# zenlc2000/pycuda-euler

Measured on AMD Instinct MI355X. Metric: k-mers/sec (encode+hash+deBruijn+Euler), 10Mx100bp k=31, 1/2/4/8 GPU, higher is better.
Workload: dtype u64

## Files before the change

### pycuda-euler_amd/csrc/assemble.hip

```cpp
#include "common.h"
#include "count_global.h"
#include "graph.h"

#include <rocprim/rocprim.hpp>

#include <algorithm>
#include <cmath>
#include <climits>
#include <cstring>
#include <cstddef>
#include <functional>
#include <type_traits>
#include <vector>

#include "count_part.h"
#include "count_v2.h"
#include "count_sk2.h"
#include "shard.h"
#include "compact.h"
#include "count_wide.h"
#include "hostin.h"
#include "join_w.h"
#include "extended.h"
#include "rank_tile.h"
// ... 166 lines not shown
    PinnedVec<uint8_t> h_lc8;
    PinnedVec<uint32_t> h_links32;
    bool links_compact = false;
    HostBuf h_blk;
    bool want_dict = false;
    hipEvent_t ev[2 * EC_NSTAGES] = {};
    hipEvent_t kev[2 * EC_NKERNELS] = {};
    bool kused[EC_NKERNELS] = {};
    bool sused[EC_NSTAGES] = {};
    bool events = false;
    bool timing = false;
    bool stage_timing = false;
    unsigned int n_dense = 0;
    bool dense_ok = false;
    bool stats_ok = false;
    unsigned flags = 0;
    DevBuf ocnt, rbc, mbid, mbid2, midx, midx2, gcur, cwalk, ewalk, lc8;
    bool no_index = false;
    uint64_t shard_base = 0;
    const uint64_t *lc_off = nullptr;
    uint64_t lc_n = 0, lc_L = 0;
    DevBuf bnp;
    DevBuf fcur, bb2;
    DevBuf nrec;
    SolidIndex gidx{};
    SolidIndexW gidxw{};
    bool graph_loaded = false;
    bool placed = false;
    uint64_t seg_lo = 0, seg_Ur = 0;
    DevBuf jrec, joid, jout, jseg, jcnt;
    DevBuf xrec;
    DevBuf skm_rec, skm_ev, skm_end;
    DevBuf wcodes_tab;
    HostBuf hmeta;
    int owner_rule = 0;
    bool own_valid = false;
    int own_rule = 0, own_nowners = 0;
    unsigned int own_n = 0, own_nblk = 0;
    std::vector<unsigned int> own_hi;
    hipStream_t cstream = nullptr;
    struct Pipe {
        bool active = false;
        bool packed = false;
        int nchunks = 0, done = 0;
        std::vector<uint64_t> blo, bhi;
        std::vector<uint64_t> ravail;
        std::vector<uint64_t> elo, ehi;
        uint64_t first_len = 0;
        const uint32_t *codes = nullptr;
        const uint64_t *exc_pos = nullptr;
        const uint8_t *exc_byte = nullptr;
        uint8_t *ascii = nullptr;
        std::vector<hipEvent_t> ev;
    } pipe;
    DevBuf p_codes, p_exc;
    struct Staged {
        Pipe pipe;
        DevBuf codes, exc, off;
        hipEvent_t free_ev = nullptr;
        uint64_t nreads = 0, nbases = 0;
    } stg[2];
    int stg_head = 0, stg_n = 0;
    bool xalpha = false;
    XAlpha xa{};
    DevBuf x_par, x_irr, x_in, x_succ, x_done, x_lk, x_lv, x_lk2, x_lv2, x_len, x_m, x_cid, x_head, x_tail;
    DevBuf jl_kof, jl_rs, jl_re, jl_cnt, jl_off, jl_flag;
    DevBuf rpack;
    DevBuf rt_tcnt, rt_tbase, rt_srec, rt_snrec, rt_sidx, rt_pks, rt_rks, rt_hasp, rt_lr;
    int spec_rounds = 0;
    DevBuf wbv;
    uint64_t seg_n0 = 0, seg_n1 = 0;
    struct Pending {
        int kind = 0;
        uint64_t n = 0;
        unsigned int ntiles = 0;
        bool planned = false;
    } hold;
    SuperRec *chain_scr = nullptr;
    unsigned int seg_nc = 0;
    uint64_t seg_nchars = 0;
    DevBuf run_cnt, run_ends, run_dends;
    DevBuf rt_lb;
    unsigned long long lb_epoch = 0;
    uint64_t run_nr = 0, run_nch = 0, run_nends = 0;
    bool runs_ready = false;
    int part_stage = 0;
    bool clip_ok = false;
    const char *clip_why = "a new session holds no assembly";
    SolidIndex cidx{};
    SolidIndexW cidxw{};
    DevBuf clip_cand, clip_list, clip_kill, clip_tot;
    DevBuf pop_key, pop_sum, pop_tcnt, pop_toff, pop_tile;
    DevBuf spec_hist;
};

static const char *const CLIP_WHY_STEPWISE =
    "the last calls were stepwise ones (ec_count_shard / ec_merge_owned* / ec_graph_*), which leave no one-GPU assembly";

static inline void drop_step_state(ec_session *s) {
    s->hold.kind = 0;
    s->runs_ready = false;
    s->chain_scr = nullptr;
    s->part_stage = 0;
}

namespace {
constexpr size_t BOUNCE_CAP = 64 << 10, BOUNCE_MAX = 16 << 10;

int d2h(ec_session *s, void *dst, const void *src, size_t n, hipStream_t st) {
    if (!n) return EC_OK;
    const size_t off = (s->bused + 15) & ~size_t(15);
    if (n > BOUNCE_MAX || off + n > BOUNCE_CAP) {
        EC_HIP(hipMemcpyAsync(dst, src, n, hipMemcpyDeviceToHost, st));
        return EC_OK;
    }
    if (!s->bounce.p) EC_CHECK(s->bounce.resize(BOUNCE_CAP));
    EC_HIP(hipMemcpyAsync(s->bounce.p + off, src, n, hipMemcpyDeviceToHost, st));
    s->pend.push_back({dst, off, n});
    s->bused = off + n;
    return EC_OK;
}

int host_wait(ec_session *s, hipEvent_t ev) {
    const hipError_t e = hipEventSynchronize(ev);
    for (const auto &q : s->pend) std::memcpy(q.dst, s->bounce.p + q.off, q.n);
    s->pend.clear();
    s->bused = 0;
    if (e != hipSuccess) {
        set_error("HIP error %s", hipGetErrorString(e));
        return EC_ERR_HIP;
    }
    return EC_OK;
}

int host_sync(ec_session *s, hipStream_t st) {
    const hipError_t e = hipStreamSynchronize(st);
    for (const auto &q : s->pend) std::memcpy(q.dst, s->bounce.p + q.off, q.n);
    s->pend.clear();
    s->bused = 0;
    if (e != hipSuccess) {
        set_error("HIP error %s", hipGetErrorString(e));
        return EC_ERR_HIP;
    }
    return EC_OK;
}
}

namespace ec {

template <typename Ops>
__global__ void __launch_bounds__(256) k_kmers_to_agg(const char *chars, const unsigned int *counts, uint64_t n, int k,
                                                      typename RecOf<typename Ops::K>::T *out, unsigned long long *bad) {
    using K = typename Ops::K;
    const K mask = Ops::mask(k);
    for (uint64_t t = blockIdx.x * (uint64_t)blockDim.x + threadIdx.x; t < n; t += (uint64_t)gridDim.x * blockDim.x) {
        const char *x = chars + t * (uint64_t)k;
        K code{};
        bool ok = true;
        for (int i = 0; i < k; i++) {
            const uint32_t b = base_code((unsigned char)x[i]);
            ok &= b < 4;
            code = Ops::push(code, b & 3u, mask);
        }
        if (!ok) atomicMin(bad, (unsigned long long)t);
        const K tw = Ops::twin(code, k);
        out[t] = RecOf<K>::make(code < tw ? code : tw, code <= tw ? counts[t] : 0u,
// ... 2036 lines not shown
    const unsigned int *SIDX = sidx ? sidx : s->rt_sidx.as<unsigned int>();
    const size_t cap = std::max<size_t>(M, 1);
    EC_CHECK(s->rt_snrec.ensure(cap * sizeof(SNodeRec)));
    EC_CHECK(s->rt_hasp.ensure(cap));
    EC_CHECK(s->rt_pks.ensure(cap * 4));
    EC_CHECK(s->rt_rks.ensure(cap * 4));
    EC_CHECK(s->rid.ensure(cap * 8));
    EC_CHECK(s->rlist.ensure(cap * 4));
    EC_CHECK(s->nextR.ensure(cap * 4));
    EC_CHECK(s->st0.ensure(cap * sizeof(RJump)));
    EC_CHECK(s->st1.ensure(cap * sizeof(RJump)));
    EC_CHECK(s->rbc.ensure(((cap + RULER_CHUNK - 1) / RULER_CHUNK) * 8 + 8));
    SNodeRec *snrec = s->rt_snrec.as<SNodeRec>();
    if (!pre_init) EC_HIP(hipMemsetAsync(s->rt_hasp.p, 0, M, st));
    k_super_link<<<grid_for(M, B), B, 0, st>>>(srec, M, SIDX, snrec, s->rt_hasp.as<uint8_t>());
    if (!pre_init) {
        EC_HIP(hipMemsetAsync(s->rid.p, 0xFF, (size_t)M * 8, st));
        EC_HIP(hipMemsetAsync(&dsc->nr, 0, 4, st));
        EC_HIP(hipMemsetAsync(&dsc->nvisited, 0, 8, st));
    }
    const unsigned int masks[4] = {15u, 3u, 1u, 0u};
    unsigned int r0 = 0;
    const unsigned int nblk = (M + RULER_CHUNK - 1) / RULER_CHUNK;
    for (int it = 0; it < 4; it++) {
        k_srulers_count<<<nblk, B, 0, st>>>(s->rt_hasp.as<uint8_t>(), M, masks[it], it == 0, s->rid.as<uint2>(),
                                            s->rbc.as<unsigned int>());
        EC_CHECK(scan_incl_u32(s, s->rbc.as<unsigned int>(), s->rbc.as<unsigned int>() + nblk, nblk));
        k_srulers<<<nblk, B, 0, st>>>(s->rt_hasp.as<uint8_t>(), M, masks[it], it == 0, s->rbc.as<unsigned int>() + nblk,
                                      &dsc->nr, s->rid.as<uint2>(), s->rlist.as<unsigned int>());
        k_rulers_total<<<1, 1, 0, st>>>(s->rbc.as<unsigned int>() + nblk, nblk, &dsc->nr);
        k_walk_s<<<2048, B, 0, st>>>(snrec, s->rlist.as<unsigned int>(), r0, &dsc->nr, masks[it], s->rid.as<uint2>(),
                                     s->nextR.as<unsigned int>(), s->st0.as<RJump>(), &dsc->nvisited, srec);
        EC_CHECK(d2h(s, &hsc, dsc, sizeof(Scalars), st));
        EC_CHECK(host_sync(s, st));
        r0 = hsc.nr;
        if (hsc.nvisited >= M) break;
    }
    nr = hsc.nr;
    if (hsc.nvisited != M) {
        set_error("ruling set covered %llu of %u chains", (unsigned long long)hsc.nvisited, M);
        return EC_ERR_STATE;
    }
    k_rjump_init<<<grid_for(nr, B), B, 0, st>>>(s->nextR.as<unsigned int>(), nr, s->st0.as<RJump>());
    rounds = 1;
    while ((1ull << (rounds - 1)) < (unsigned long long)nr) rounds++;
    rounds = std::min(rounds + 1, 63);
    RJump *bufs[2] = {s->st0.as<RJump>(), s->st1.as<RJump>()};
    EC_HIP(hipMemsetAsync(dsc->active, 0, sizeof(dsc->active), st));
    for (int r = 0; r < rounds; r++)
        k_rjump<<<grid_for(nr, B), B, 0, st>>>(bufs[r & 1], bufs[(r + 1) & 1], nr, N, r ? &dsc->active[r - 1] : nullptr,
                                              &dsc->active[r], &dsc->final_sel, (unsigned)((r + 1) & 1));
    k_finalize_s<<<grid_for(M, B), B, 0, st>>>(snrec, srec, s->rid.as<uint2>(), s->rlist.as<unsigned int>(), bufs[0],
                                              bufs[1], &dsc->final_sel, &dsc->active[rounds - 1], M,
                                              s->rt_pks.as<unsigned int>(), s->rt_rks.as<unsigned int>(),
                                              s->PL.as<unsigned int>(), s->PM.as<unsigned long long>());
    k_cycle_len_s<<<grid_for(nr, B), B, 0, st>>>(s->nextR.as<unsigned int>(), s->rlist.as<unsigned int>(), srec, bufs[0],
                                                bufs[1], &dsc->final_sel, &dsc->active[rounds - 1], nr,
                                                s->PL.as<unsigned int>(), s->PM.as<unsigned long long>());
    return EC_OK;
}

int rank_supers_async(ec_session *s, unsigned int N, const unsigned long long *dM, int &rounds,
                      unsigned int mcap = 0, const unsigned int *sidx = nullptr) {
    const unsigned int G = mcap ? mcap : N;
    hipStream_t st = s->stream;
    const unsigned B = 256;
    Scalars *dsc = s->scal.as<Scalars>();
    SuperRec *srec = s->rt_srec.as<SuperRec>();
    const size_t cap = mcap ? (size_t)mcap + 4096 : std::max<size_t>(N, 1);
    const unsigned int spare = mcap ? 16u : 0u;
    EC_CHECK(s->rt_snrec.ensure(cap * sizeof(SNodeRec), spare));
    EC_CHECK(s->rt_pks.ensure(cap * 4, spare));
    EC_CHECK(s->rt_rks.ensure(cap * 4, spare));
    EC_CHECK(s->rlist.ensure(cap * 4, spare));
    EC_CHECK(s->nextR.ensure(cap * 4, spare));
    EC_CHECK(s->rbc.ensure(((cap + RULER_CHUNK - 1) / RULER_CHUNK) * 8 + 8, spare));
    SNodeRec *snrec = s->rt_snrec.as<SNodeRec>();
    const unsigned int *dnr = &dsc->nr;
    const unsigned int gs = std::min(grid_for(G, B), 4096u);
    k_super_link<<<gs, B, 0, st>>>(srec, 0, sidx ? sidx : s->rt_sidx.as<unsigned int>(), snrec,
                                   s->rt_hasp.as<uint8_t>(), dM);
    const unsigned int smask = 15u;
    const unsigned int nblk = (G + RULER_CHUNK - 1) / RULER_CHUNK;
    k_srulers_count<<<nblk, B, 0, st>>>(s->rt_hasp.as<uint8_t>(), 0, smask, 1, s->rid.as<uint2>(),
                                        s->rbc.as<unsigned int>(), dM);
    EC_CHECK(scan_incl_u32(s, s->rbc.as<unsigned int>(), s->rbc.as<unsigned int>() + nblk, nblk));
    k_srulers<<<nblk, B, 0, st>>>(s->rt_hasp.as<uint8_t>(), 0, smask, 1, s->rbc.as<unsigned int>() + nblk, &dsc->nr,
                                  s->rid.as<uint2>(), s->rlist.as<unsigned int>(), dM);
    k_rulers_total<<<1, 1, 0, st>>>(s->rbc.as<unsigned int>() + nblk, nblk, &dsc->nr);
    k_walk_s<<<2048, B, 0, st>>>(snrec, s->rlist.as<unsigned int>(), 0, &dsc->nr, smask, s->rid.as<uint2>(),
                                 s->nextR.as<unsigned int>(), s->st0.as<RJump>(), &dsc->nvisited, srec);
    const unsigned int gr = std::min(grid_for(G / 8u + 1, B), 2048u);
    k_rjump_init<<<gr, B, 0, st>>>(s->nextR.as<unsigned int>(), 0, s->st0.as<RJump>(), dnr);
    rounds = 1;
    while ((1ull << (rounds - 1)) < (unsigned long long)G) rounds++;
    rounds = std::min(rounds + 1, 63);
    if (s->spec_rounds > 0 && s->spec_rounds < rounds) rounds = s->spec_rounds;
    RJump *bufs[2] = {s->st0.as<RJump>(), s->st1.as<RJump>()};
    for (int r = 0; r < rounds; r++)
        k_rjump<<<gr, B, 0, st>>>(bufs[r & 1], bufs[(r + 1) & 1], 0, N, r ? &dsc->active[r - 1] : nullptr,
                                  &dsc->active[r], &dsc->final_sel, (unsigned)((r + 1) & 1), dnr);
    k_finalize_s<<<gs, B, 0, st>>>(snrec, srec, s->rid.as<uint2>(), s->rlist.as<unsigned int>(), bufs[0], bufs[1],
                                   &dsc->final_sel, &dsc->active[rounds - 1], 0, s->rt_pks.as<unsigned int>(),
                                   s->rt_rks.as<unsigned int>(), s->PL.as<unsigned int>(),
                                   s->PM.as<unsigned long long>(), dM);
    k_cycle_len_s<<<gr, B, 0, st>>>(s->nextR.as<unsigned int>(), s->rlist.as<unsigned int>(), srec, bufs[0], bufs[1],
                                    &dsc->final_sel, &dsc->active[rounds - 1], 0, s->PL.as<unsigned int>(),
                                    s->PM.as<unsigned long long>(), dnr);
    return EC_OK;
}

__global__ void __launch_bounds__(256) k_pack_chars(const uint4 *chars, const unsigned long long *total, uint64_t cap16,
                                                    uint32_t *codes) {
    const uint64_t n16 = min<uint64_t>((*total + 15) / 16, cap16);
    for (uint64_t t = blockIdx.x * (uint64_t)blockDim.x + threadIdx.x; t < n16; t += (uint64_t)gridDim.x * blockDim.x) {
        const uint4 v = chars[t];
        const uint32_t w[4] = {v.x, v.y, v.z, v.w};
        uint32_t out = 0;
#pragma unroll
        for (int u = 0; u < 4; u++) {
            const uint32_t x = ((w[u] >> 1) ^ (w[u] >> 2)) & 0x03030303u;
            const uint32_t y = x | (x >> 6);
            out |= ((y | (y >> 12)) & 0xFFu) << (8 * u);
        }
        codes[t] = out;
    }
}

constexpr unsigned int OCOPY_MIN = 1u << 16;
int rounds_used(const Scalars &h, int rounds) {
    if (rounds <= 0 || h.active[rounds - 1]) return 0;
    int used = 1;
    for (int r = 0; r < rounds; r++)
        if (h.active[r]) used = r + 2;
    return std::min(used, rounds);
}
void note_rounds(ec_session *s, const Scalars &h, int rounds) {
    const int used = rounds_used(h, rounds);
    s->spec_rounds = used ? used + 1 : 0;
}

int x_cut(ec_session *s, unsigned int U, unsigned int &nx) {
    hipStream_t st = s->stream;
    const unsigned B = 256;
    Scalars *dsc = s->scal.as<Scalars>();
    const unsigned int N = 2 * U;
    nx = 0;
    EC_HIP(hipMemsetAsync(&dsc->nasym, 0, 16, st));
    k_x_asym<<<grid_for(N, B), B, 0, st>>>(s->upal.as<uint8_t>(), s->succ.as<unsigned int>(), N, &dsc->nasym);
    unsigned int nasym = 0;
    EC_CHECK(d2h(s, &nasym, &dsc->nasym, 4, st));
    EC_CHECK(host_sync(s, st));
    if (kn().verbose) fprintf(stderr, "extended: %u one-way links among %u nodes\n", nasym, N);
    if (!nasym) return EC_OK;
    EC_CHECK(s->x_par.ensure((size_t)U * 4));
    EC_CHECK(s->x_irr.ensure(U));
    EC_CHECK(s->x_in.ensure(U));
    EC_CHECK(s->x_succ.ensure((size_t)N * 4));
    EC_CHECK(s->x_lk.ensure((size_t)N * 8));
    EC_CHECK(s->x_lk2.ensure((size_t)N * 8));
    EC_CHECK(s->x_lv.ensure((size_t)N * 4));
    EC_CHECK(s->x_lv2.ensure((size_t)N * 4));
    unsigned int *par = s->x_par.as<unsigned int>(), *tree = s->x_lv2.as<unsigned int>();
    k_x_iota<<<grid_for(U, B), B, 0, st>>>(tree, U);
    k_x_uf_link<<<grid_for(N, B), B, 0, st>>>(s->upal.as<uint8_t>(), s->succ.as<unsigned int>(), N, tree);
    k_x_uf_flatten<<<grid_for(U, B), B, 0, st>>>(U, tree, par);
    EC_HIP(hipMemsetAsync(s->x_irr.p, 0, U, st));
    k_x_mark_irr<<<grid_for(N, B), B, 0, st>>>(s->upal.as<uint8_t>(), s->succ.as<unsigned int>(), N, par,
                                              s->x_irr.as<uint8_t>());
    k_x_cut<<<grid_for(N, B), B, 0, st>>>(s->upal.as<uint8_t>(), N, par, s->x_irr.as<uint8_t>(), s->x_in.as<uint8_t>(),
                                         s->succ.as<unsigned int>(), s->x_succ.as<unsigned int>(),
                                         s->dfc.as<unsigned long long>(), s->dft.as<unsigned long long>(),
// ... 1223 lines not shown
    for (uint64_t i = 0; i < n_exc; i++)
        if (exc_pos[i] >= nbases || (i && exc_pos[i] <= exc_pos[i - 1])) {
            set_error("exception %llu: position %llu not ascending inside [0, %llu)", (unsigned long long)i,
                      (unsigned long long)exc_pos[i], (unsigned long long)nbases);
            return EC_ERR_ARG;
        }
    return EC_OK;
}

int stage_packed(ec_session *s, Pipe &pp, DevBuf &codes_b, DevBuf &exc_b, DevBuf &off_b, hipEvent_t after,
                 const uint8_t *codes, uint64_t nbases, const uint64_t *offsets, uint64_t nreads, uint32_t read_len,
                 const uint64_t *exc_pos, const uint8_t *exc_byte, uint64_t n_exc) {
    const uint64_t ncodes = (nbases + 3) / 4;
    EC_CHECK(off_b.ensure((nreads + 1) * 8));
    EC_CHECK(codes_b.ensure(((ncodes + 3) & ~3ull) + 16));
    EC_CHECK(exc_b.ensure(n_exc * 9 + 16));
    EC_CHECK(pipe_plan(s, pp, nbases, 1, offsets, nreads, read_len, after));
    pp.packed = true;
    pp.first_len = nreads ? (offsets ? offsets[1] - offsets[0] : read_len) : 0;
    pp.codes = codes_b.as<uint32_t>();
    pp.exc_pos = exc_b.as<uint64_t>();
    pp.exc_byte = exc_b.as<uint8_t>() + n_exc * 8;
    if (n_exc) {
        EC_HIP(hipMemcpyAsync(exc_b.p, exc_pos, n_exc * 8, hipMemcpyHostToDevice, s->cstream));
        EC_HIP(hipMemcpyAsync(exc_b.as<uint8_t>() + n_exc * 8, exc_byte, n_exc, hipMemcpyHostToDevice, s->cstream));
    }
    if (!offsets)
        k_iota_off<<<grid_for(nreads + 1, 256, 16384), 256, 0, s->cstream>>>(off_b.as<uint64_t>(), nreads + 1, read_len);
    for (int c = 0; c < pp.nchunks; c++) {
        const uint64_t c0 = pp.blo[c] / 4, c1 = c + 1 == pp.nchunks ? ncodes : pp.bhi[c] / 4;
        if (c1 > c0)
            EC_HIP(hipMemcpyAsync(codes_b.as<uint8_t>() + c0, codes + c0, c1 - c0, hipMemcpyHostToDevice, s->cstream));
        if (offsets) EC_CHECK(pipe_copy_offsets(s, pp, c, offsets, off_b.as<uint64_t>()));
        pp.elo[c] = (uint64_t)(std::lower_bound(exc_pos, exc_pos + n_exc, pp.blo[c]) - exc_pos);
        pp.ehi[c] = (uint64_t)(std::lower_bound(exc_pos, exc_pos + n_exc, pp.bhi[c]) - exc_pos);
        EC_HIP(hipEventRecord(pp.ev[c], s->cstream));
    }
    return EC_OK;
}

}

static void unpack_codes(const uint8_t *codes, uint64_t n, char *out) {
    static const struct Lut {
        uint32_t v[256];
        Lut() {
            const char acgt[4] = {'A', 'C', 'G', 'T'};
            for (int b = 0; b < 256; b++) {
                uint32_t w = 0;
                for (int j = 0; j < 4; j++) w |= (uint32_t)(uint8_t)acgt[(b >> (2 * j)) & 3] << (8 * j);
                v[b] = w;
            }
        }
    } lut;
    auto run = [&](uint64_t b0, uint64_t b1) {
        for (uint64_t i = b0; i < b1; i++) memcpy(out + 4 * i, &lut.v[codes[i]], 4);
    };
    const uint64_t full = n / 4;
    const unsigned nt = full >= (1ull << 20) ? std::max(1u, std::min(16u, std::thread::hardware_concurrency())) : 1u;
    if (nt > 1) {
        std::vector<std::thread> th;
        for (unsigned t = 0; t < nt; t++) th.emplace_back(run, full * t / nt, full * (t + 1) / nt);
        for (auto &x : th) x.join();
    } else {
        run(0, full);
    }
    for (uint64_t c = 4 * full; c < n; c++) out[c] = "ACGT"[(codes[full] >> (2 * (c & 3))) & 3];
}

template <typename Fn>
static void for_each_buf(ec_session *s, Fn fn) {
    DevBuf *all[] = {&s->h_reads, &s->h_offsets, &s->hll, &s->scal, &s->table, &s->dkey, &s->dcnt, &s->dfc, &s->dft,
                     &s->upal, &s->outdeg, &s->cand, &s->succ, &s->pred, &s->st0, &s->st1, &s->startOf, &s->skeys,
                     &s->svals, &s->skeys2, &s->svals2, &s->cidxOf, &s->clen, &s->coff, &s->chars, &s->cfirst,
                     &s->clast, &s->headOf, &s->tailOf, &s->lk, &s->lcnt, &s->tmp, &s->dchars, &s->dcounts,
                     &s->rid, &s->rlist, &s->nextR, &s->PK, &s->RK, &s->PL, &s->PM,
                     &s->ocnt, &s->hist, &s->ftot, &s->cnt, &s->offs, &s->bstart, &s->tot, &s->recs, &s->recs2, &s->sub, &s->bnp, &s->rbc,
                     &s->mbid, &s->mbid2, &s->midx, &s->midx2, &s->gcur, &s->cwalk, &s->ewalk, &s->lc8, &s->x_par, &s->x_irr,
                     &s->x_in, &s->x_succ, &s->x_done, &s->x_lk, &s->x_lv, &s->x_lk2, &s->x_lv2, &s->x_len,
                     &s->x_m, &s->x_cid, &s->x_head, &s->x_tail, &s->rt_tcnt, &s->rt_tbase, &s->rt_srec,
                     &s->rt_snrec, &s->rt_sidx, &s->rt_pks, &s->rt_rks, &s->rt_hasp, &s->rt_lr, &s->wbv, &s->bmark, &s->rt_tb,
                     &s->jrec, &s->joid, &s->jout, &s->jseg, &s->jcnt, &s->xrec,
                     &s->skm_rec, &s->skm_ev, &s->skm_end, &s->wcodes_tab,
                     &s->run_cnt, &s->run_ends, &s->run_dends, &s->rt_lb,
                     &s->jl_kof, &s->jl_rs, &s->jl_re, &s->jl_cnt, &s->jl_off, &s->jl_flag, &s->jl_frec, &s->rpack,
                     &s->clip_cand, &s->clip_list, &s->clip_kill, &s->clip_tot,
                     &s->pop_key, &s->pop_sum, &s->pop_tcnt, &s->pop_toff, &s->pop_tile, &s->spec_hist};
    for (auto *b : all) fn(*b);
}

extern "C" {

int ec_session_create(ec_session **out, int device) {
    if (!out) {
        set_error("null out");
        return EC_ERR_ARG;
    }
    int n = 0;
    EC_HIP(hipGetDeviceCount(&n));
    if (device < 0 || device >= n) {
        set_error("device %d not in [0,%d)", device, n);
        return EC_ERR_ARG;
    }
    EC_HIP(hipSetDevice(device));
    ec_session *s = new ec_session();
    s->device = device;
    if (hipStreamCreateWithFlags(&s->stream, hipStreamNonBlocking) != hipSuccess) {
        delete s;
        set_error("hipStreamCreate failed");
        return EC_ERR_HIP;
    }
    s->own_stream = true;
    *out = s;
    return EC_OK;
}

int ec_session_set_stream(ec_session *s, void *hip_stream) {
    if (!s) return EC_ERR_ARG;
    EC_HIP(hipSetDevice(s->device));
    if (hip_stream == EC_OWN_STREAM) {
        if (!s->own_stream) {
            EC_HIP(hipStreamCreateWithFlags(&s->stream, hipStreamNonBlocking));
            s->own_stream = true;
        }
        return EC_OK;
    }
    if (s->own_stream && s->stream) {
        (void)host_sync(s, s->stream);
        hipStreamDestroy(s->stream);
    }
    s->own_stream = false;
    s->stream = (hipStream_t)hip_stream;
    return EC_OK;
}

uint64_t ec_session_bytes(ec_session *s) {
    uint64_t n = 0;
    if (s) for_each_buf(s, [&](DevBuf &b) { n += b.cap; });
    return n;
}

int ec_session_trim(ec_session *s, uint64_t min_bytes) {
    if (!s) return EC_ERR_ARG;
    EC_HIP(hipSetDevice(s->device));
    if (s->stream) EC_HIP(hipStreamSynchronize(s->stream));
    if (s->ostream) EC_HIP(hipStreamSynchronize(s->ostream));
    if (s->cstream) EC_HIP(hipStreamSynchronize(s->cstream));
    for_each_buf(s, [&](DevBuf &b) {
        if (b.cap >= min_bytes && &b != &s->scal) b.release();
    });
    drop_step_state(s);
    s->n_dense = 0;
    s->dense_ok = false;
    s->clip_ok = false;
    s->clip_why = "ec_session_trim released the assembly's device state";
    s->own_valid = false;
    s->bmark_ok = false;
    s->seg_marks = 0;
    s->skspec.valid = false;
    s->jlspec.valid = s->jlspec.queued = false;
    s->graph_loaded = false;
    s->placed = false;
    s->pipe.active = false;
    return EC_OK;
}

int ec_mem_stats(uint64_t *held, uint64_t *peak, int reset) {
// ... 1402 lines not shown
```

### pycuda-euler_amd/csrc/graph.h

```cpp
#pragma once
#include "count_global.h"
#include "count_part.h"
#include "superkmer.h"
#include "wide.h"

namespace ec {

struct SolidIndex {
    const Slot *table;
    uint64_t capmask;
    const SubSlot *sub;
    int bbits;
    unsigned int slots;
    int sk;
    const uint8_t *npb;
    int pmax;
    MinCfg mc;
    int bijk = 0;
    __device__ inline unsigned int find_in(uint64_t c, unsigned int h, uint64_t b) const {
        const SubSlot *r = sub + b * slots;
        unsigned int n = slots;
        if (npb) {
            n = slots >> pmax;
            r += ((h >> 11) & ((1u << npb[b]) - 1)) * n;
// ... 356 lines not shown
            const unsigned int i = off + (unsigned int)__popcll(m & ((1ull << lane) - 1));
            rlist[i] = (unsigned int)t;
            rid[t] = make_uint2(i, 0u);
        }
        base += tot;
        __syncthreads();
    }
}

__global__ void k_rulers_total(const unsigned int *bs, unsigned int nblk, unsigned int *nr) { *nr += bs[nblk - 1]; }

struct alignas(32) RJump {
    unsigned int a;
    unsigned int s;
    unsigned int h;
    unsigned int cm;
    unsigned int cd;
    unsigned int len;
    unsigned long long fm;
};
static_assert(sizeof(RJump) == 32, "rjump layout");


__global__ void __launch_bounds__(256) k_walk(const NodeRec *nrec, const unsigned int *rlist,
                                              unsigned int r0, const unsigned int *nr, unsigned int smask,
                                              uint2 *rid, unsigned int *nextR, RJump *rs,
                                              unsigned long long *nvisited) {
    const unsigned int r1 = *nr;
    unsigned long long seen = 0;
    for (uint64_t t = r0 + blockIdx.x * (uint64_t)blockDim.x + threadIdx.x; t < r1; t += (uint64_t)gridDim.x * blockDim.x) {
        const unsigned int i = (unsigned int)t;
        unsigned int v = rlist[i];
        const NodeRec a = nrec[v];
        unsigned long long fm = a.fev;
        unsigned int j = 0, nx = NONE32;
        unsigned int w = a.succ;
        for (;;) {
            if (w == NONE32) break;
            if (ruler_hash(w, smask)) {
                const unsigned int q = rid[w].x;
                if (q != NONE32) {
                    nx = q;
                    break;
                }
            }
            v = w;
            j++;
            const NodeRec b = nrec[v];
            w = b.succ;
            rid[v] = make_uint2(i, j);
            fm = b.fev < fm ? b.fev : fm;
        }
        nextR[i] = nx;
        RJump r;
        r.a = NONE32;
        r.s = 0;
        r.h = i;
        r.cm = rlist[i];
        r.cd = 0;
        r.len = j + 1;
        r.fm = fm;
        rs[i] = r;
        seen += j + 1;
    }
    for (int o = 32; o > 0; o >>= 1) seen += __shfl_down(seen, o);
    __shared__ unsigned long long bseen[4];
    if ((threadIdx.x & 63) == 0) bseen[threadIdx.x >> 6] = seen;
    __syncthreads();
    if (threadIdx.x == 0) {
        const unsigned long long v = bseen[0] + bseen[1] + bseen[2] + bseen[3];
        if (v) atomicAdd(nvisited, v);
    }
}

__global__ void __launch_bounds__(256) k_rjump_init(const unsigned int *nextR, unsigned int nr, RJump *rs,
                                                    const unsigned int *dnr = nullptr) {
    if (dnr) nr = *dnr;
    for (uint64_t t = blockIdx.x * (uint64_t)blockDim.x + threadIdx.x; t < nr; t += (uint64_t)gridDim.x * blockDim.x) {
        const unsigned int n = nextR[t];
        if (n != NONE32) rs[n].a = (unsigned int)t;
    }
}

__global__ void __launch_bounds__(256) k_rjump(const RJump *src, RJump *dst, unsigned int nr, unsigned int N,
                                               const unsigned int *active_in, unsigned int *active_out,
                                               unsigned int *final_sel, unsigned int sel,
                                               const unsigned int *dnr = nullptr) {
    if (active_in && *active_in == 0) return;
    if (dnr) nr = *dnr;
    unsigned int act = 0;
    auto take = [&](RJump &j, const RJump &y) {
        const unsigned int back = j.s + y.len;
        if (y.cm < j.cm) {
            j.cm = y.cm;
            j.cd = back + y.cd;
        }
        const unsigned long long s2 = (unsigned long long)back + y.s;
        j.s = s2 < 0xFFFFFFFFull ? (unsigned int)s2 : 0xFFFFFFFFu;
        j.a = y.a;
        j.h = y.h;
        j.fm = y.fm < j.fm ? y.fm : j.fm;
    };
    for (uint64_t t = blockIdx.x * (uint64_t)blockDim.x + threadIdx.x; t < nr; t += (uint64_t)gridDim.x * blockDim.x) {
        RJump j = src[t];
        if (j.a != NONE32 && j.s < N) {
            take(j, src[j.a]);
            if (j.a != NONE32 && j.s < N) take(j, src[j.a]);
            act += (j.a != NONE32 && j.s < N);
        }
        dst[t] = j;
    }
    if (__syncthreads_or(act != 0) && threadIdx.x == 0) *active_out = 1u;
    if (blockIdx.x == 0 && threadIdx.x == 0) *final_sel = sel;
}

constexpr unsigned int CYC = 0x80000000u;

__global__ void __launch_bounds__(256) k_finalize(const uint8_t *upal, const unsigned int *succ, const uint2 *rid,
                                                  const unsigned int *rlist, const RJump *rs0, const RJump *rs1,
                                                  const unsigned int *sel, const unsigned int *unconverged,
                                                  unsigned int N, unsigned int *PK,
                                                  unsigned int *RK, unsigned int *PL, unsigned long long *PM) {
    if (*unconverged) {
        for (uint64_t t = blockIdx.x * (uint64_t)blockDim.x + threadIdx.x; t < N; t += (uint64_t)gridDim.x * blockDim.x) {
            PK[t] = (unsigned int)t;
            RK[t] = 0;
            PL[t] = 1;
            PM[t] = 0;
        }
        return;
    }
    const RJump *rs = (*sel & 1) ? rs1 : rs0;
    for (uint64_t t = blockIdx.x * (uint64_t)blockDim.x + threadIdx.x; t < N; t += (uint64_t)gridDim.x * blockDim.x) {
        const unsigned int x = (unsigned int)t;
        if ((x & 1) && upal[x >> 1]) continue;
        const uint2 ro = rid[x];
        const unsigned int i = ro.x, j = ro.y;
        const RJump r = rs[i];
        if (r.a == NONE32) {
            const unsigned int pk = rlist[r.h], rk = r.s + j;
            PK[x] = pk;
            RK[x] = rk;
            if (succ[x] == NONE32) {
                PL[pk] = rk + 1;
                PM[pk] = r.fm;
            }
        } else {
            PK[x] = r.cm | CYC;
            RK[x] = r.cd + j;
        }
    }
}

__global__ void __launch_bounds__(256) k_cycle_len(const unsigned int *nextR, const unsigned int *rlist,
                                                   const RJump *rs0, const RJump *rs1, const unsigned int *sel,
                                                   const unsigned int *unconverged, unsigned int nr, unsigned int *PL,
                                                   unsigned long long *PM) {
    if (*unconverged) return;
    const RJump *rs = (*sel & 1) ? rs1 : rs0;
    for (uint64_t t = blockIdx.x * (uint64_t)blockDim.x + threadIdx.x; t < nr; t += (uint64_t)gridDim.x * blockDim.x) {
        const RJump r = rs[t];
        if (r.a == NONE32) continue;
        const unsigned int n = nextR[t];
        if (n != NONE32 && rlist[n] == r.cm) {
            PL[r.cm] = r.cd + r.len;
            PM[r.cm] = r.fm;
        }
    }
}

struct PathOf {
    const unsigned int *PK, *RK;
    const unsigned int *LH, *LR, *PKs, *RKs;
    __device__ inline unsigned int pk(unsigned int x) const {
        if (LH) {
            const unsigned int h = LH[x];
            if (!(h & 0x80000000u)) return PKs[h];
        }
        return PK[x];
    }
    __device__ inline void get(unsigned int x, unsigned int &pk, unsigned int &rk) const {
        if (LH) {
            const unsigned int h = LH[x];
            if (!(h & 0x80000000u)) {
                pk = PKs[h];
                rk = RKs[h] + LR[x];
                return;
            }
        }
        pk = PK[x];
// ... 400 lines not shown
```

### pycuda-euler_amd/csrc/rank_tile.h

```cpp
#pragma once

#include "graph.h"

namespace ec {

constexpr int RT_TN = 2048;
constexpr int RT_NT = 512;
constexpr int RT_PER = RT_TN / RT_NT;
constexpr int RT_ROUNDS = 11;
constexpr unsigned int RT_FIN = 0x80000000u;
constexpr uint16_t RT_NONE = 0xFFFFu;

struct alignas(16) SuperRec {
    unsigned int head, succ, w, pad;
    unsigned long long fmin;
    unsigned long long pad2;
};
struct alignas(16) SNodeRec {
    unsigned int succ;
    unsigned int w;
    unsigned long long fev;
};

struct TileLB {
// ... 302 lines not shown
        *nr = 0;
        *nvisited = 0;
    }
    if (nchains && t == 0 && threadIdx.x == 0) *nchains = tbase[gridDim.x];
}

__global__ void __launch_bounds__(256) k_part_rank_init(unsigned long long *dM, unsigned int M, uint8_t *hasp, uint2 *rid,
                                                        unsigned int *nr, unsigned long long *nvisited) {
    if (blockIdx.x == 0 && threadIdx.x == 0) *dM = M, *nr = 0, *nvisited = 0;
    for (uint64_t t = blockIdx.x * (uint64_t)blockDim.x + threadIdx.x; t < M; t += (uint64_t)gridDim.x * blockDim.x) {
        hasp[t] = 0;
        rid[t] = make_uint2(NONE32, NONE32);
    }
}

__global__ void __launch_bounds__(256) k_super_index(const SuperRec *srec, unsigned int M, unsigned int *SIDX) {
    for (uint64_t t = blockIdx.x * (uint64_t)blockDim.x + threadIdx.x; t < M; t += (uint64_t)gridDim.x * blockDim.x)
        SIDX[srec[t].head] = (unsigned int)t;
}

__global__ void __launch_bounds__(256) k_super_link(const SuperRec *srec, unsigned int M, const unsigned int *SIDX,
                                                    SNodeRec *nrec, uint8_t *hasp,
                                                    const unsigned long long *dM = nullptr) {
    if (dM) M = (unsigned int)*dM;
    for (uint64_t t = blockIdx.x * (uint64_t)blockDim.x + threadIdx.x; t < M; t += (uint64_t)gridDim.x * blockDim.x) {
        const SuperRec r = srec[t];
        const unsigned int s = r.succ == NONE32 ? NONE32 : SIDX[r.succ];
        SNodeRec o;
        o.succ = s;
        o.w = r.w;
        o.fev = r.fmin;
        nrec[t] = o;
        if (s != NONE32) hasp[s] = 1;
    }
}

__device__ inline bool sruler_sel(const uint8_t *hasp, const uint2 *rid, unsigned int i, unsigned int smask,
                                  int first) {
    if (rid[i].x != NONE32) return false;
    return (first && !hasp[i]) || ruler_hash(i, smask);
}
__global__ void __launch_bounds__(256) k_srulers_count(const uint8_t *hasp, unsigned int M, unsigned int smask,
                                                       int first, const uint2 *rid, unsigned int *bc,
                                                       const unsigned long long *dM = nullptr) {
    if (dM) M = (unsigned int)*dM;
    const uint64_t c0 = (uint64_t)blockIdx.x * RULER_CHUNK;
    const uint64_t c1 = c0 + RULER_CHUNK < M ? c0 + RULER_CHUNK : M;
    unsigned int c = 0;
    for (uint64_t t = c0 + threadIdx.x; t < c1; t += blockDim.x) c += sruler_sel(hasp, rid, (unsigned int)t, smask, first);
    for (int o = 32; o > 0; o >>= 1) c += __shfl_xor(c, o);
    __shared__ unsigned int w[4];
    if ((threadIdx.x & 63) == 0) w[threadIdx.x >> 6] = c;
    __syncthreads();
    if (threadIdx.x == 0) bc[blockIdx.x] = w[0] + w[1] + w[2] + w[3];
}
__global__ void __launch_bounds__(256) k_srulers(const uint8_t *hasp, unsigned int M, unsigned int smask, int first,
                                                 const unsigned int *bs, const unsigned int *nr, uint2 *rid,
                                                 unsigned int *rlist, const unsigned long long *dM = nullptr) {
    if (dM) M = (unsigned int)*dM;
    __shared__ unsigned int wsum[4];
    const uint64_t c0 = (uint64_t)blockIdx.x * RULER_CHUNK;
    const uint64_t c1 = c0 + RULER_CHUNK < M ? c0 + RULER_CHUNK : M;
    unsigned int base = *nr + (blockIdx.x ? bs[blockIdx.x - 1] : 0u);
    const unsigned int lane = threadIdx.x & 63, wid = threadIdx.x >> 6;
    for (uint64_t t0 = c0; t0 < c1; t0 += blockDim.x) {
        const uint64_t t = t0 + threadIdx.x;
        const bool sel = t < c1 && sruler_sel(hasp, rid, (unsigned int)t, smask, first);
        const unsigned long long m = __ballot(sel);
        if (lane == 0) wsum[wid] = (unsigned int)__popcll(m);
        __syncthreads();
        unsigned int off = base;
        for (unsigned int q = 0; q < wid; q++) off += wsum[q];
        const unsigned int tot = wsum[0] + wsum[1] + wsum[2] + wsum[3];
        if (sel) {
            const unsigned int i = off + (unsigned int)__popcll(m & ((1ull << lane) - 1));
            rlist[i] = (unsigned int)t;
            rid[t] = make_uint2(i, 0u);
        }
        base += tot;
        __syncthreads();
    }
}

__global__ void __launch_bounds__(256) k_walk_s(const SNodeRec *nrec, const unsigned int *rlist, unsigned int r0,
                                                const unsigned int *nr, unsigned int smask, uint2 *rid,
                                                unsigned int *nextR, RJump *rs, unsigned long long *nvisited,
                                                const SuperRec *srec) {
    const unsigned int r1 = *nr;
    unsigned long long seen = 0;
    for (uint64_t t = r0 + blockIdx.x * (uint64_t)blockDim.x + threadIdx.x; t < r1; t += (uint64_t)gridDim.x * blockDim.x) {
        const unsigned int i = (unsigned int)t;
        unsigned int v = rlist[i];
        const SNodeRec a = nrec[v];
        unsigned long long fm = a.fev;
        unsigned int j = 0, wl = a.w, cnt = 1, nx = NONE32;
        unsigned int w = a.succ;
        for (;;) {
            if (w == NONE32) break;
            if (ruler_hash(w, smask)) {
                const unsigned int q = rid[w].x;
                if (q != NONE32) {
                    nx = q;
                    break;
                }
            }
            v = w;
            j += wl;
            const SNodeRec b = nrec[v];
            w = b.succ;
            wl = b.w;
            rid[v] = make_uint2(i, j);
            fm = b.fev < fm ? b.fev : fm;
            cnt++;
        }
        nextR[i] = nx;
        RJump r;
        r.a = NONE32;
        r.s = 0;
        r.h = srec[rlist[i]].head;
        r.cm = rlist[i];
        r.cd = 0;
        r.len = j + wl;
        r.fm = fm;
        rs[i] = r;
        seen += cnt;
    }
    for (int o = 32; o > 0; o >>= 1) seen += __shfl_down(seen, o);
    __shared__ unsigned long long bseen[4];
    if ((threadIdx.x & 63) == 0) bseen[threadIdx.x >> 6] = seen;
    __syncthreads();
    if (threadIdx.x == 0) {
        const unsigned long long v = bseen[0] + bseen[1] + bseen[2] + bseen[3];
        if (v) atomicAdd(nvisited, v);
    }
}

__global__ void __launch_bounds__(256) k_finalize_s(const SNodeRec *nrec, const SuperRec *srec, const uint2 *rid,
                                                    const unsigned int *rlist, const RJump *rs0, const RJump *rs1,
                                                    const unsigned int *sel, const unsigned int *unconverged,
                                                    unsigned int M, unsigned int *PKs, unsigned int *RKs,
                                                    unsigned int *PL, unsigned long long *PM,
                                                    const unsigned long long *dM = nullptr) {
    if (dM) M = (unsigned int)*dM;
    const bool bad = *unconverged != 0;
    const RJump *rs = (*sel & 1) ? rs1 : rs0;
    for (uint64_t t = blockIdx.x * (uint64_t)blockDim.x + threadIdx.x; t < M; t += (uint64_t)gridDim.x * blockDim.x) {
        const unsigned int v = (unsigned int)t;
        const uint2 ro = rid[v];
        if (bad || ro.x == NONE32) {
            PKs[v] = srec[v].head;
            RKs[v] = 0;
            continue;
        }
        const RJump r = rs[ro.x];
        if (r.a == NONE32) {
            const unsigned int pk = r.h, rk = r.s + ro.y;
            PKs[v] = pk;
            RKs[v] = rk;
            if (nrec[v].succ == NONE32) {
                PL[pk] = rk + nrec[v].w;
                PM[pk] = r.fm;
            }
        } else {
            PKs[v] = srec[r.cm].head | CYC;
            RKs[v] = r.cd + ro.y;
        }
// ... 97 lines not shown
```

Before: 204.7 billion.

## Fuse ruler selection into single-pass lookback kernel and deepen rjump hops

Replaces the ruler count kernel, device scan and scatter kernel, plus the single-thread total kernel, with one kernel that uses decoupled tile lookback over an epoch-tagged status buffer to compute global offsets in a single pass. This removes three launches and a full second read of hasp/rid. Separately, each pointer-jumping round in k_rjump now takes up to four hops instead of two. The number of rounds is unchanged, so the extra hops add dependent gathers per round without reducing launches unless the round count is also tuned. The lookback relies on forward progress across blocks.

```diff
diff --git a/pycuda-euler_amd/csrc/assemble.hip b/pycuda-euler_amd/csrc/assemble.hip
--- a/pycuda-euler_amd/csrc/assemble.hip
+++ b/pycuda-euler_amd/csrc/assemble.hip
@@ -272,6 +272,8 @@
     DevBuf run_cnt, run_ends, run_dends;
     DevBuf rt_lb;
     unsigned long long lb_epoch = 0;
+    DevBuf rl_lb;
+    unsigned long long rl_epoch = 0;
     uint64_t run_nr = 0, run_nch = 0, run_nends = 0;
     bool runs_ready = false;
     int part_stage = 0;
@@ -2474,12 +2476,20 @@
                                    s->rt_hasp.as<uint8_t>(), dM);
     const unsigned int smask = 15u;
     const unsigned int nblk = (G + RULER_CHUNK - 1) / RULER_CHUNK;
-    k_srulers_count<<<nblk, B, 0, st>>>(s->rt_hasp.as<uint8_t>(), 0, smask, 1, s->rid.as<uint2>(),
-                                        s->rbc.as<unsigned int>(), dM);
-    EC_CHECK(scan_incl_u32(s, s->rbc.as<unsigned int>(), s->rbc.as<unsigned int>() + nblk, nblk));
-    k_srulers<<<nblk, B, 0, st>>>(s->rt_hasp.as<uint8_t>(), 0, smask, 1, s->rbc.as<unsigned int>() + nblk, &dsc->nr,
-                                  s->rid.as<uint2>(), s->rlist.as<unsigned int>(), dM);
-    k_rulers_total<<<1, 1, 0, st>>>(s->rbc.as<unsigned int>() + nblk, nblk, &dsc->nr);
+    {
+        const size_t oldcap = s->rl_lb.cap;
+        EC_CHECK(s->rl_lb.ensure(((size_t)nblk + 1) * 8, spare));
+        s->rl_epoch = (s->rl_epoch + 1) & ((1ull << 30) - 1);
+        if (s->rl_lb.cap != oldcap || s->rl_epoch == 0) {
+            EC_HIP(hipMemsetAsync(s->rl_lb.p, 0, s->rl_lb.cap, st));
+            s->rl_epoch = 1;
+        }
+    }
+    TileLB rlb{};
+    rlb.status = s->rl_lb.as<unsigned long long>();
+    rlb.epoch = s->rl_epoch;
+    k_srulers_lb<<<nblk, B, 0, st>>>(s->rt_hasp.as<uint8_t>(), smask, s->rid.as<uint2>(), s->rlist.as<unsigned int>(), dM,
+                                     rlb, &dsc->nr);
     k_walk_s<<<2048, B, 0, st>>>(snrec, s->rlist.as<unsigned int>(), 0, &dsc->nr, smask, s->rid.as<uint2>(),
                                  s->nextR.as<unsigned int>(), s->st0.as<RJump>(), &dsc->nvisited, srec);
     const unsigned int gr = std::min(grid_for(G / 8u + 1, B), 2048u);
@@ -3869,7 +3879,7 @@
                      &s->rt_snrec, &s->rt_sidx, &s->rt_pks, &s->rt_rks, &s->rt_hasp, &s->rt_lr, &s->wbv, &s->bmark, &s->rt_tb,
                      &s->jrec, &s->joid, &s->jout, &s->jseg, &s->jcnt, &s->xrec,
                      &s->skm_rec, &s->skm_ev, &s->skm_end, &s->wcodes_tab,
-                     &s->run_cnt, &s->run_ends, &s->run_dends, &s->rt_lb,
+                     &s->run_cnt, &s->run_ends, &s->run_dends, &s->rt_lb, &s->rl_lb,
                      &s->jl_kof, &s->jl_rs, &s->jl_re, &s->jl_cnt, &s->jl_off, &s->jl_flag, &s->jl_frec, &s->rpack,
                      &s->clip_cand, &s->clip_list, &s->clip_kill, &s->clip_tot,
                      &s->pop_key, &s->pop_sum, &s->pop_tcnt, &s->pop_toff, &s->pop_tile, &s->spec_hist};
diff --git a/pycuda-euler_amd/csrc/graph.h b/pycuda-euler_amd/csrc/graph.h
--- a/pycuda-euler_amd/csrc/graph.h
+++ b/pycuda-euler_amd/csrc/graph.h
@@ -462,6 +462,7 @@
     }
 }
 
+constexpr int RJ_HOPS = 4;
 __global__ void __launch_bounds__(256) k_rjump(const RJump *src, RJump *dst, unsigned int nr, unsigned int N,
                                                const unsigned int *active_in, unsigned int *active_out,
                                                unsigned int *final_sel, unsigned int sel,
@@ -485,7 +486,9 @@
         RJump j = src[t];
         if (j.a != NONE32 && j.s < N) {
             take(j, src[j.a]);
-            if (j.a != NONE32 && j.s < N) take(j, src[j.a]);
+#pragma unroll
+            for (int h = 1; h < RJ_HOPS; h++)
+                if (j.a != NONE32 && j.s < N) take(j, src[j.a]);
             act += (j.a != NONE32 && j.s < N);
         }
         dst[t] = j;
diff --git a/pycuda-euler_amd/csrc/rank_tile.h b/pycuda-euler_amd/csrc/rank_tile.h
--- a/pycuda-euler_amd/csrc/rank_tile.h
+++ b/pycuda-euler_amd/csrc/rank_tile.h
@@ -408,6 +408,62 @@
     }
 }
 
+__global__ void __launch_bounds__(256) k_srulers_lb(const uint8_t *hasp, unsigned int smask, uint2 *rid,
+                                                    unsigned int *rlist, const unsigned long long *dM, TileLB lb,
+                                                    unsigned int *nr) {
+    constexpr unsigned int ITERS = RULER_CHUNK / 256;
+    static_assert(ITERS * 4 == 64, "a wave sums the chunk's per-wave counts");
+    __shared__ unsigned int s_cnt[ITERS][4];
+    __shared__ unsigned int s_base;
+    const unsigned int M = (unsigned int)*dM;
+    const uint64_t c0 = (uint64_t)blockIdx.x * RULER_CHUNK;
+    if (c0 >= M && blockIdx.x) return;
+    const uint64_t c1 = c0 + RULER_CHUNK < M ? c0 + RULER_CHUNK : M;
+    const unsigned int lane = threadIdx.x & 63, wid = threadIdx.x >> 6;
+    unsigned int rx[ITERS];
+    uint8_t hp[ITERS];
+#pragma unroll
+    for (unsigned int it = 0; it < ITERS; it++) {
+        const uint64_t t = c0 + (uint64_t)it * 256 + threadIdx.x;
+        rx[it] = t < c1 ? rid[t].x : 0u;
+        hp[it] = t < c1 ? hasp[t] : (uint8_t)1;
+    }
+    unsigned int selbits = 0;
+#pragma unroll
+    for (unsigned int it = 0; it < ITERS; it++) {
+        const uint64_t t = c0 + (uint64_t)it * 256 + threadIdx.x;
+        const bool sel = t < c1 && rx[it] == NONE32 && (!hp[it] || ruler_hash((unsigned int)t, smask));
+        selbits |= (unsigned int)sel << it;
+        const unsigned long long m = __ballot(sel);
+        if (lane == 0) s_cnt[it][wid] = (unsigned int)__popcll(m);
+    }
+    __syncthreads();
+    if (wid == 0) {
+        unsigned int tot = (&s_cnt[0][0])[lane];
+        for (int o = 32; o > 0; o >>= 1) tot += __shfl_xor(tot, o);
+        const unsigned long long g = tile_lookback(lb, blockIdx.x, tot, lane);
+        if (lane == 0) {
+            s_base = (unsigned int)g;
+            if (c0 + RULER_CHUNK >= M) *nr = (unsigned int)g + tot;
+        }
+    }
+    __syncthreads();
+    unsigned int base = s_base;
+    for (unsigned int it = 0; it < ITERS; it++) {
+        const bool sel = (selbits >> it) & 1u;
+        const unsigned long long m = __ballot(sel);
+        unsigned int off = base;
+        for (unsigned int q = 0; q < wid; q++) off += s_cnt[it][q];
+        base += s_cnt[it][0] + s_cnt[it][1] + s_cnt[it][2] + s_cnt[it][3];
+        if (sel) {
+            const uint64_t t = c0 + (uint64_t)it * 256 + threadIdx.x;
+            const unsigned int i = off + (unsigned int)__popcll(m & ((1ull << lane) - 1));
+            rlist[i] = (unsigned int)t;
+            rid[t] = make_uint2(i, 0u);
+        }
+    }
+}
+
 __global__ void __launch_bounds__(256) k_walk_s(const SNodeRec *nrec, const unsigned int *rlist, unsigned int r0,
                                                 const unsigned int *nr, unsigned int smask, uint2 *rid,
                                                 unsigned int *nextR, RJump *rs, unsigned long long *nvisited,
```

After: 199.4 billion. -2.6%, worse.
